# Itseez/opencv

Hardware: AMD Instinct MI355X
Metric: Mpix/s per GPU (4K CV_8U Gaussian5x5) + achieved HBM GB/s vs roofline, 1/2/4/8 GPUs (higher is better)
Workload: dtype u8; 1 GPU; cv::GaussianBlur 5x5 sigma=0 BORDER_REFLECT_101 on 3840x2160 CV_8UC1, 9216 device-resident frames per GPU per step (152.9 GB of HBM: one pass = 18 launches of 512 frames); frames_per_gpu=9216, frames_per_launch=512, ranks=1, collective=none (1 GPU)

## Files before the change

opencv_amd/csrc/smooth.hip:

```cpp
#include "rt.h"
#include "gausskernel.h"
#include "seproll.h"
#include "seplong.h"
#include "sepmx.h"
#include <cstring>
#include <cstdlib>

using namespace mi355;

namespace {

struct FixedTaps { uint16_t kx[33]; uint16_t ky[33]; int nx, ny; };

__global__ __launch_bounds__(256) void k_sepfixed_generic(
    const uchar* __restrict__ src, size_t sstep, size_t sframe,
    uchar* __restrict__ dst, size_t dstep, size_t dframe,
    int W, int H, int cn, int mL, int mT, int mR, int mB, int border, FixedTaps t)
{
    const int b = blockIdx.x * 64 + (threadIdx.x & 63);
    const int y = blockIdx.y * 4 + (threadIdx.x >> 6);
    if (b >= W * cn || y >= H) return;
    src += (size_t)blockIdx.z * sframe;
    dst += (size_t)blockIdx.z * dframe;
    const int x = b / cn, c = b - x * cn;
    const int fullW = mL + W + mR, fullH = mT + H + mB;
    const int rx = t.nx / 2, ry = t.ny / 2;
    uint32_t acc = 0;
    for (int j = 0; j < t.ny; j++) {
        int yy = mi355_borderInterpolate(y + mT + j - ry, fullH, border);
        if (yy < 0) continue;
        const uchar* row = src + (ptrdiff_t)(yy - mT) * (ptrdiff_t)sstep;
        uint32_t h = 0;
        for (int i = 0; i < t.nx; i++) {
            int xx = mi355_borderInterpolate(x + mL + i - rx, fullW, border);
            if (xx < 0) continue;
            h += (uint32_t)t.kx[i] * row[(ptrdiff_t)(xx - mL) * cn + c];
        }
        h = h > 0xFFFFu ? 0xFFFFu : h;
        uint64_t a = (uint64_t)acc + (uint64_t)t.ky[j] * h;
        acc = a > 0xFFFFFFFFull ? 0xFFFFFFFFu : (uint32_t)a;
    }
    uint32_t r = (uint32_t)(((uint64_t)acc + 0x8000u) >> 16);
    dst[(size_t)y * dstep + b] = (uchar)(r > 255 ? 255 : r);
}

constexpr int floordiv2(int a) { return a >= 0 ? a / 2 : -((-a + 1) / 2); }
constexpr int mod2(int a) { return ((a % 2) + 2) % 2; }

template <int Q, int S, int HD>
__device__ __forceinline__ uint32_t pairAt(const uint32_t* E, const uint32_t* O, int k)
{
    constexpr int q2 = mod2(Q + S);
    constexpr int f = floordiv2(Q + S);
    const uint32_t* P = q2 ? O : E;
    if constexpr (mod2(f) == 0) {
        return P[k + f / 2 + HD];
    } else {
        constexpr int lo = floordiv2(f - 1) + 0;
        return __builtin_amdgcn_alignbit(P[k + lo + 1 + HD], P[k + lo + HD], 16);
    }
}

template <int HD> struct RawRow {
    uint4 m;
    uint32_t hl[HD];
    uint32_t hr[HD];
};

template <int KS, int CN> struct RollCfg {
    static constexpr int R = KS / 2;
    static constexpr int HB = R * CN;
    static constexpr int HD = (HB + 3) / 4;
};

template <int KS, int CN>
__device__ __forceinline__ void loadRow(RawRow<RollCfg<KS, CN>::HD>& r, const uchar* __restrict__ src, size_t sstep,
                                        int yy, int W, int H, int c, int nchunks, int lane, int border)
{
    constexpr int HD = RollCfg<KS, CN>::HD, HB = RollCfg<KS, CN>::HB;
    r.m = make_uint4(0, 0, 0, 0);
#pragma unroll
    for (int d = 0; d < HD; d++) { r.hl[d] = 0; r.hr[d] = 0; }
    const int ry = mi355_borderInterpolate(yy, H, border);
    if (ry < 0 || c >= nchunks) return;
    const uchar* row = src + (size_t)ry * sstep;
    r.m = *reinterpret_cast<const uint4*>(row + 16 * (size_t)c);
    if (lane == 0) {
        if (c > 0) {
#pragma unroll
            for (int d = 0; d < HD; d++) r.hl[d] = *reinterpret_cast<const uint32_t*>(row + 16 * (size_t)c - 4 * (HD - d));
        } else {
#pragma unroll
            for (int t = -HB; t < 0; t++) {
                const int px = (t - (CN - 1)) / CN;
                const int ch = t - px * CN;
                const int sp = mi355_borderInterpolate(px, W, border);
                const uint32_t v = sp < 0 ? 0u : row[sp * CN + ch];
                r.hl[(4 * HD + t) >> 2] |= v << (8 * ((4 * HD + t) & 3));
            }
        }
    }
    if (c == nchunks - 1) {
#pragma unroll
        for (int t = 0; t < HB; t++) {
            const int px = W + t / CN, ch = t % CN;
            const int sp = mi355_borderInterpolate(px, W, border);
            const uint32_t v = sp < 0 ? 0u : row[sp * CN + ch];
            r.hr[t >> 2] |= v << (8 * (t & 3));
        }
    } else if (lane == 63) {
#pragma unroll
        for (int d = 0; d < HD; d++) r.hr[d] = *reinterpret_cast<const uint32_t*>(row + 16 * (size_t)c + 16 + 4 * d);
    }
}

template <int KS, int CN>
__device__ __forceinline__ void hfilter(uint32_t (&Hrow)[8], const RawRow<RollCfg<KS, CN>::HD>& r, int c, int nchunks, int lane)
{
    constexpr int HD = RollCfg<KS, CN>::HD;
    constexpr int NW = 4 + 2 * HD;
    uint32_t X[NW];
    const uint32_t mv[4] = {r.m.x, r.m.y, r.m.z, r.m.w};
#pragma unroll
    for (int d = 0; d < HD; d++) {
        uint32_t l = __shfl_up(mv[4 - HD + d], 1);
        uint32_t rr = __shfl_down(mv[d], 1);
        X[d] = (lane == 0) ? r.hl[d] : l;
        X[HD + 4 + d] = (lane == 63 || c == nchunks - 1) ? r.hr[d] : rr;
    }
#pragma unroll
    for (int d = 0; d < 4; d++) X[HD + d] = mv[d];
    uint32_t E[NW], O[NW];
#pragma unroll
    for (int d = 0; d < NW; d++) {
        E[d] = __builtin_amdgcn_perm(0u, X[d], 0x0c020c00u);
        O[d] = __builtin_amdgcn_perm(0u, X[d], 0x0c030c01u);
    }
#pragma unroll
    for (int k = 0; k < 4; k++) {
        if constexpr (KS == 5) {
            {   uint32_t a = pairAt<0, -2 * CN, HD>(E, O, k) + pairAt<0, 2 * CN, HD>(E, O, k);
                uint32_t b = pairAt<0, -CN, HD>(E, O, k) + pairAt<0, CN, HD>(E, O, k);
                uint32_t m = pairAt<0, 0, HD>(E, O, k);
                Hrow[k] = a + (b << 2) + (m << 1) + (m << 2); }
            {   uint32_t a = pairAt<1, -2 * CN, HD>(E, O, k) + pairAt<1, 2 * CN, HD>(E, O, k);
                uint32_t b = pairAt<1, -CN, HD>(E, O, k) + pairAt<1, CN, HD>(E, O, k);
                uint32_t m = pairAt<1, 0, HD>(E, O, k);
                Hrow[4 + k] = a + (b << 2) + (m << 1) + (m << 2); }
        } else {
            Hrow[k]     = pairAt<0, -CN, HD>(E, O, k) + pairAt<0, CN, HD>(E, O, k) + (pairAt<0, 0, HD>(E, O, k) << 1);
            Hrow[4 + k] = pairAt<1, -CN, HD>(E, O, k) + pairAt<1, CN, HD>(E, O, k) + (pairAt<1, 0, HD>(E, O, k) << 1);
        }
    }
}

template <int KS, int CN>
__global__ __launch_bounds__(256) void k_binomial_roll(
    const uchar* __restrict__ src, size_t sstep, size_t sframe,
    uchar* __restrict__ dst, size_t dstep, size_t dframe,
    int W, int H, int nchunks, int segRows, int border)
{
    constexpr int R = KS / 2, HD = RollCfg<KS, CN>::HD;
    const int lane = threadIdx.x & 63;
    const int c = (blockIdx.x * 4 + (threadIdx.x >> 6)) * 64 + lane;
    const int y0 = blockIdx.y * segRows;
    const int y1 = min(H, y0 + segRows);
    src += (size_t)blockIdx.z * sframe;
    dst += (size_t)blockIdx.z * dframe;
    const bool active = c < nchunks;

    uint32_t Hw[KS][8];
    {
        RawRow<HD> pre[KS - 1];
#pragma unroll
        for (int i = 0; i < KS - 1; i++) loadRow<KS, CN>(pre[i], src, sstep, y0 - R + i, W, H, c, nchunks, lane, border);
#pragma unroll
        for (int i = 0; i < KS - 1; i++) hfilter<KS, CN>(Hw[i], pre[i], c, nchunks, lane);
    }
    for (int y = y0; y < y1; y += KS) {
        RawRow<HD> raw[KS];
#pragma unroll
        for (int u = 0; u < KS; u++)
            if (y + u < y1) loadRow<KS, CN>(raw[u], src, sstep, y + u + R, W, H, c, nchunks, lane, border);
#pragma unroll
        for (int u = 0; u < KS; u++) {
            if (y + u < y1) {
                hfilter<KS, CN>(Hw[(KS - 1 + u) % KS], raw[u], c, nchunks, lane);
                uint32_t o[4];
                if constexpr (KS == 5) {
                    const uint32_t* h0 = Hw[(u + 0) % 5]; const uint32_t* h1 = Hw[(u + 1) % 5];
                    const uint32_t* h2 = Hw[(u + 2) % 5]; const uint32_t* h3 = Hw[(u + 3) % 5];
                    const uint32_t* h4 = Hw[(u + 4) % 5];
                    uint32_t v[8];
#pragma unroll
                    for (int i = 0; i < 8; i++) {
                        const uint32_t b4 = lshlAdd(h1[i] + h3[i] + h2[i], 2, 0x00800080u);
                        v[i] = h0[i] + h4[i] + lshlAdd(h2[i], 1, b4);
                    }
#pragma unroll
                    for (int k = 0; k < 4; k++) o[k] = __builtin_amdgcn_perm(v[4 + k], v[k], 0x07030501u);
                } else {
                    const uint32_t* h0 = Hw[(u + 0) % 3]; const uint32_t* h1 = Hw[(u + 1) % 3]; const uint32_t* h2 = Hw[(u + 2) % 3];
#pragma unroll
                    for (int k = 0; k < 4; k++) {
                        uint32_t ve = ((h0[k] + h2[k] + (h1[k] << 1) + 0x00080008u) >> 4) & 0x00FF00FFu;
                        uint32_t vo = ((h0[4 + k] + h2[4 + k] + (h1[4 + k] << 1) + 0x00080008u) >> 4) & 0x00FF00FFu;
                        o[k] = ve | (vo << 8);
                    }
                }
                if (active)
                    *reinterpret_cast<uint4*>(dst + (size_t)(y + u) * dstep + 16 * (size_t)c) = make_uint4(o[0], o[1], o[2], o[3]);
            }
        }
    }
}

template <int HD> struct RawRow2 {
    uint4 m;
    uint32_t side[HD];
};

template <int HD> struct EdgeSel {
    uint32_t la[HD], lb[HD], lc[HD];
    uint32_t ra[HD], rb[HD], rc[HD];
};

__device__ __forceinline__ void selSetByte(uint32_t& a, uint32_t& b, uint32_t& c, int j, int idx )
{
    const uint32_t sh = 8u * (uint32_t)j, clr = ~(0xffu << sh);
    uint32_t va = 0x0cu, vb = 0x0cu, vc = 0x0cu;
    if (idx >= 8)      { vb = (uint32_t)(idx - 8); vc = 4u + (uint32_t)j; }
    else if (idx >= 0) { va = (uint32_t)idx;       vc = (uint32_t)j; }
    a = (a & clr) | (va << sh); b = (b & clr) | (vb << sh); c = (c & clr) | (vc << sh);
}

__device__ __forceinline__ uint32_t gather16(const uint4& m, uint32_t a, uint32_t b, uint32_t c)
{
    const uint32_t t1 = __builtin_amdgcn_perm(m.y, m.x, a);
    const uint32_t t2 = __builtin_amdgcn_perm(m.w, m.z, b);
    return __builtin_amdgcn_perm(t2, t1, c);
}

template <int KS, int CN, bool NTL = false>
__device__ __forceinline__ void issueRow(RawRow2<RollCfg<KS, CN>::HD>& r, const uchar* __restrict__ row, int mainOff, int sideOff)
{
    constexpr int HD = RollCfg<KS, CN>::HD;
    if constexpr (NTL) {
        typedef uint32_t u32x4 __attribute__((ext_vector_type(4)));
        u32x4 v = __builtin_nontemporal_load(reinterpret_cast<const u32x4*>(row + mainOff));
        r.m = make_uint4(v.x, v.y, v.z, v.w);
    } else
    r.m = *reinterpret_cast<const uint4*>(row + mainOff);
#pragma unroll
    for (int d = 0; d < HD; d++) r.side[d] = *reinterpret_cast<const uint32_t*>(row + sideOff + 4 * d);
}

template <int KS, int CN, bool EB = true>
__device__ __forceinline__ void hfilter2(uint32_t (&Hrow)[8], const RawRow2<RollCfg<KS, CN>::HD>& r,
                                         bool hasFirst, bool hasLast, bool isLastChunk, const EdgeSel<RollCfg<KS, CN>::HD>& es)
{
    constexpr int HD = RollCfg<KS, CN>::HD;
    constexpr int NW = 4 + 2 * HD;
    uint32_t X[NW];
    const uint32_t mv[4] = {r.m.x, r.m.y, r.m.z, r.m.w};
    uint32_t hl[HD], hr[HD];
#pragma unroll
    for (int d = 0; d < HD; d++) { hl[d] = r.side[d]; hr[d] = r.side[d]; }
    if (hasFirst) {
#pragma unroll
        for (int d = 0; d < HD; d++) { hl[d] = gather16(r.m, es.la[d], es.lb[d], es.lc[d]); if constexpr (EB) asm volatile("" : "+v"(hl[d])); }
    }
    uint32_t hb[HD];
#pragma unroll
    for (int d = 0; d < HD; d++) hb[d] = 0;
    if (hasLast) {
#pragma unroll
        for (int d = 0; d < HD; d++) { hb[d] = gather16(r.m, es.ra[d], es.rb[d], es.rc[d]); if constexpr (EB) asm volatile("" : "+v"(hb[d])); }
    }
#pragma unroll
    for (int d = 0; d < HD; d++) {
        X[d] = __builtin_amdgcn_update_dpp(hl[d], mv[4 - HD + d], 0x138, 0xf, 0xf, false);
        uint32_t rr = __builtin_amdgcn_update_dpp(hr[d], mv[d], 0x130, 0xf, 0xf, false);
        if (hasLast) { rr = isLastChunk ? hb[d] : rr; if constexpr (EB) asm volatile("" : "+v"(rr)); }
        X[HD + 4 + d] = rr;
    }
#pragma unroll
    for (int d = 0; d < 4; d++) X[HD + d] = mv[d];
    uint32_t E[NW], O[NW];
#pragma unroll
    for (int d = 0; d < NW; d++) {
        E[d] = __builtin_amdgcn_perm(0u, X[d], 0x0c020c00u);
        O[d] = __builtin_amdgcn_perm(0u, X[d], 0x0c030c01u);
    }
#pragma unroll
    for (int k = 0; k < 4; k++) {
        if constexpr (KS == 5) {
            {   uint32_t a = pairAt<0, -2 * CN, HD>(E, O, k) + pairAt<0, 2 * CN, HD>(E, O, k);
                uint32_t b = pairAt<0, -CN, HD>(E, O, k) + pairAt<0, CN, HD>(E, O, k);
                uint32_t m = pairAt<0, 0, HD>(E, O, k);
                Hrow[k] = a + (b << 2) + (m << 1) + (m << 2); }
            {   uint32_t a = pairAt<1, -2 * CN, HD>(E, O, k) + pairAt<1, 2 * CN, HD>(E, O, k);
                uint32_t b = pairAt<1, -CN, HD>(E, O, k) + pairAt<1, CN, HD>(E, O, k);
                uint32_t m = pairAt<1, 0, HD>(E, O, k);
                Hrow[4 + k] = a + (b << 2) + (m << 1) + (m << 2); }
        } else {
            Hrow[k]     = pairAt<0, -CN, HD>(E, O, k) + pairAt<0, CN, HD>(E, O, k) + (pairAt<0, 0, HD>(E, O, k) << 1);
            Hrow[4 + k] = pairAt<1, -CN, HD>(E, O, k) + pairAt<1, CN, HD>(E, O, k) + (pairAt<1, 0, HD>(E, O, k) << 1);
        }
    }
}

template <int KS, int CN, bool NT, bool NTL, int WPS, bool EB = true>
__global__ __launch_bounds__(256, WPS) void k_binomial_roll2(
    const uchar* __restrict__ src, size_t sstep, size_t sframe,
    uchar* __restrict__ dst, size_t dstep, size_t dframe,
    int W, int H, int nchunks, int nstrips, int segRows, int nseg, int nframes, int border, int alt)
{
    constexpr int R = KS / 2, HD = RollCfg<KS, CN>::HD, HB = RollCfg<KS, CN>::HB;
    const int lane = threadIdx.x & 63;
    const int wid = __builtin_amdgcn_readfirstlane((int)(blockIdx.x * 4 + (threadIdx.x >> 6)));
    const int strip = wid % nstrips;
    const int t0 = wid / nstrips;
    int seg = t0 % nseg;
    const int frame = t0 / nseg;
    if (frame >= nframes) return;
    int up = 0;
    if (alt) {
        const int G = 1 << alt, span = 8 * G;
        const int g = seg / span, j = seg - g * span;
        if ((g + 1) * span <= nseg) seg = g * span + G * (j & 7) + (j >> 3);
        else if (alt > 1) {
            const int base = g * span, t = seg - base, g2 = t >> 4, j2 = t & 15;
            if (base + (g2 << 4) + 16 <= nseg) seg = base + (g2 << 4) + 2 * (j2 & 7) + (j2 >> 3);
        }
        up = seg & 1;
    }
    const int c = strip * 64 + lane;
    const int y0 = seg * segRows;
    const int y1 = min(H, y0 + segRows);
    src += (size_t)frame * sframe;
    dst += (size_t)frame * dframe;
    const bool active = c < nchunks;
    const bool hasFirst = strip == 0, hasLast = strip == nstrips - 1;
    const bool isLastChunk = c == nchunks - 1;
    const int ce = active ? c : nchunks - 1;
    const int mainOff = 16 * ce;
    const int c0 = strip * 64;
    const int leftOff = c0 > 0 ? 16 * c0 - 4 * HD : 0;
    const int rightOff = c0 + 64 < nchunks ? 16 * (c0 + 64) : 16 * (nchunks - 1);
    const int sideOff = lane < 32 ? leftOff : rightOff;

    EdgeSel<HD> es;
#pragma unroll
    for (int d = 0; d < HD; d++) { es.la[d] = es.lb[d] = es.lc[d] = es.ra[d] = es.rb[d] = es.rc[d] = 0x0c0c0c0cu; }
    if (hasFirst) {
#pragma unroll
        for (int t = 0; t < HB; t++) {
            const int bt = t - HB;
            const int px = (bt - (CN - 1)) / CN;
            const int sp = mi355_borderInterpolate(px, W, border);
            const int pos = 4 * HD - HB + t;
            selSetByte(es.la[pos >> 2], es.lb[pos >> 2], es.lc[pos >> 2], pos & 3, sp < 0 ? -1 : sp * CN + (bt - px * CN));
        }
    }
    if (hasLast) {
#pragma unroll
        for (int t = 0; t < HB; t++) {
            const int sp = mi355_borderInterpolate(W + t / CN, W, border);
            selSetByte(es.ra[t >> 2], es.rb[t >> 2], es.rc[t >> 2], t & 3, sp < 0 ? -1 : sp * CN + (t % CN) - 16 * (nchunks - 1));
        }
    }
    int rowBelow[R], rowAbove[R];
#pragma unroll
    for (int i = 0; i < R; i++) { rowBelow[i] = mi355_borderInterpolate(H + i, H, border); rowAbove[i] = mi355_borderInterpolate(-1 - i, H, border); }
    const int nrows = y1 - y0;
    auto gy = [&](int j) -> int { return up ? y1 - 1 - j : y0 + j; };
    auto rowIdx = [&](int g) -> int {
        int ry = g;
#pragma unroll
        for (int i = 0; i < R; i++) { ry = (g == H + i) ? rowBelow[i] : ry; ry = (g == -1 - i) ? rowAbove[i] : ry; }
        return ry;
    };

    uint32_t Hw[KS][8];
#pragma unroll
    for (int i = 0; i < KS - 1; i++) {
        const int ry = rowIdx(gy(min(i - R, nrows - 1 + R)));
        if (ry < 0) {
#pragma unroll
            for (int j = 0; j < 8; j++) Hw[i][j] = 0;
        } else {
            RawRow2<HD> pre;
            issueRow<KS, CN>(pre, src + (size_t)ry * sstep, mainOff, sideOff);
            hfilter2<KS, CN, EB>(Hw[i], pre, hasFirst, hasLast, isLastChunk, es);
        }
    }
    RawRow2<HD> raw[KS];
    int rvalid[KS];
#pragma unroll
    for (int u = 0; u < KS; u++) {
        const int ry = rowIdx(gy(min(u + R, nrows - 1 + R)));
        rvalid[u] = ry >= 0;
        issueRow<KS, CN, NTL>(raw[u], src + (size_t)max(ry, 0) * sstep, mainOff, sideOff);
    }
    for (int y = 0; y < nrows; y += KS) {
#pragma unroll
        for (int u = 0; u < KS; u++) {
            if (y + u < nrows) {
                uint32_t (&Hn)[8] = Hw[(KS - 1 + u) % KS];
                if (rvalid[u]) hfilter2<KS, CN, EB>(Hn, raw[u], hasFirst, hasLast, isLastChunk, es);
                else {
#pragma unroll
                    for (int j = 0; j < 8; j++) Hn[j] = 0;
                }
                {
                    const int ry = rowIdx(gy(min(y + u + KS + R, nrows - 1 + R)));
                    rvalid[u] = ry >= 0;
                    issueRow<KS, CN, NTL>(raw[u], src + (size_t)max(ry, 0) * sstep, mainOff, sideOff);
                }
                uint32_t o[4];
                if constexpr (KS == 5) {
                    const uint32_t* h0 = Hw[(u + 0) % 5]; const uint32_t* h1 = Hw[(u + 1) % 5];
                    const uint32_t* h2 = Hw[(u + 2) % 5]; const uint32_t* h3 = Hw[(u + 3) % 5];
                    const uint32_t* h4 = Hw[(u + 4) % 5];
                    uint32_t v[8];
#pragma unroll
                    for (int i = 0; i < 8; i++) {
                        if constexpr (EB) {
                            const uint32_t b4 = lshlAdd(h1[i] + h3[i] + h2[i], 2, 0x00800080u);
                            v[i] = h0[i] + h4[i] + lshlAdd(h2[i], 1, b4);
                        } else
                            v[i] = (h0[i] + h4[i]) + ((h1[i] + h3[i]) << 2) + (h2[i] << 1) + (h2[i] << 2) + 0x00800080u;
                    }
#pragma unroll
                    for (int k = 0; k < 4; k++) o[k] = __builtin_amdgcn_perm(v[4 + k], v[k], 0x07030501u);
                } else {
                    const uint32_t* h0 = Hw[(u + 0) % 3]; const uint32_t* h1 = Hw[(u + 1) % 3]; const uint32_t* h2 = Hw[(u + 2) % 3];
#pragma unroll
                    for (int k = 0; k < 4; k++) {
                        uint32_t ve = ((h0[k] + h2[k] + (h1[k] << 1) + 0x00080008u) >> 4) & 0x00FF00FFu;
                        uint32_t vo = ((h0[4 + k] + h2[4 + k] + (h1[4 + k] << 1) + 0x00080008u) >> 4) & 0x00FF00FFu;
                        o[k] = ve | (vo << 8);
                    }
                }
                if (active) {
                    typedef uint32_t u32x4 __attribute__((ext_vector_type(4)));
                    u32x4 ov = {o[0], o[1], o[2], o[3]};
                    u32x4* dp = reinterpret_cast<u32x4*>(dst + (size_t)gy(y + u) * dstep + 16 * (size_t)c);
                    if constexpr (NT) __builtin_nontemporal_store(ov, dp);
                    else *dp = ov;
                }
            }
        }
    }
}

template <bool NT>
__global__ __launch_bounds__(256) void k_copy16(const uint4* __restrict__ s, uint4* __restrict__ d, size_t n16, int perThread)
{
    typedef uint32_t u32x4 __attribute__((ext_vector_type(4)));
    size_t base = ((size_t)blockIdx.x * perThread) * 256 + threadIdx.x;
#pragma unroll 4
    for (int i = 0; i < perThread; i++) {
        size_t j = base + (size_t)i * 256;
        if (j < n16) {
            uint4 v = s[j];
            u32x4 ov = {v.x, v.y, v.z, v.w};
            if constexpr (NT) __builtin_nontemporal_store(ov, reinterpret_cast<u32x4*>(d + j));
            else d[j] = v;
        }
    }
}

template <int UNROLL>
__global__ __launch_bounds__(256) void k_copy_colwalk(const uchar* __restrict__ src, uchar* __restrict__ dst, size_t step, size_t frame,
                                                      int H, int nchunks, int nstrips, int segRows, int nseg, int nframes)
{
    const int lane = threadIdx.x & 63;
    const int wid = __builtin_amdgcn_readfirstlane((int)(blockIdx.x * 4 + (threadIdx.x >> 6)));
    const int strip = wid % nstrips, t0 = wid / nstrips, seg = t0 % nseg, fr = t0 / nseg;
    if (fr >= nframes) return;
    const int c = strip * 64 + lane;
    if (c >= nchunks) return;
    const int y0 = seg * segRows, y1 = min(H, y0 + segRows);
    const uchar* s = src + (size_t)fr * frame + 16 * (size_t)c;
    uchar* d = dst + (size_t)fr * frame + 16 * (size_t)c;
    for (int y = y0; y < y1; y += UNROLL) {
        uint4 v[UNROLL];
#pragma unroll
        for (int u = 0; u < UNROLL; u++) v[u] = *reinterpret_cast<const uint4*>(s + (size_t)min(y + u, y1 - 1) * step);
#pragma unroll
        for (int u = 0; u < UNROLL; u++) if (y + u < y1) *reinterpret_cast<uint4*>(d + (size_t)(y + u) * step) = v[u];
    }
}


bool aligned16(const void* p, size_t step) { return (((uintptr_t)p | step) & 15) == 0; }

int envInt(const char* n, int d) { const char* v = getenv(n); return v ? atoi(v) : d; }

int& tuneSeg() { static int v = envInt("MI355CV_GAUSS_SEG", 0); return v; }
int& tuneVariant() { static int v = envInt("MI355CV_GAUSS_VARIANT", 3); return v; }

int& tuneAlt() { static int v = envInt("MI355CV_GAUSS_ALT", 1); return v; }
int& tuneLaunchWaves() { static int v = envInt("MI355CV_GAUSS_LAUNCH_WAVES", 393216); return v; }

template <int KS, int CN>
void launchRoll2(const uchar* s, size_t ss, size_t sf, uchar* d, size_t ds, size_t df, int nframes, int W, int H, int border, hipStream_t st, int nt)
{
    const int nchunks = W * CN / 16;
    const int nstrips = divUp(nchunks, 64);
    int seg = tuneSeg();
    if (seg <= 0) {
        long long per = (long long)nstrips * nframes;
        long long wantSeg = (2048 + per - 1) / per;
        seg = (int)((H + wantSeg - 1) / wantSeg);
        const int best = 16;
        if (seg > best) seg = best;
        if (seg < KS) seg = KS;
    }
    if (seg > H) seg = H;
    const int nseg = divUp(H, seg);
    const long long perFrame = (long long)nstrips * nseg;
    long long chunk = tuneLaunchWaves() > 0 ? (tuneLaunchWaves() + perFrame - 1) / perFrame : nframes;
    if (chunk < 1) chunk = 1;
    if (chunk > nframes) chunk = nframes;
    const int nlaunch = (int)((nframes + chunk - 1) / chunk);
    noteKernel("k_binomial_roll2<%d,%d,%s,false,%d,%s> grid=%u x256 seg=%d rows alt=%d, %d launch(es) of <= %lld frames", KS, CN, nt >= 1 ? "true" : "false", nt == 3 ? 6 : 4,
               nt == 2 ? "false" : "true", (unsigned)((perFrame * chunk + 3) / 4), seg, tuneAlt(), nlaunch, chunk);
    for (long long f0 = 0; f0 < nframes; f0 += chunk) {
        const int nf = (int)(nframes - f0 < chunk ? nframes - f0 : chunk);
        const uchar* sp = s + (size_t)f0 * sf;
        uchar* dp = d + (size_t)f0 * df;
        dim3 grid((unsigned)((perFrame * nf + 3) / 4));
        if (nt == 3)      hipLaunchKernelGGL((k_binomial_roll2<KS, CN, true, false, 6>), grid, dim3(256), 0, st, sp, ss, sf, dp, ds, df, W, H, nchunks, nstrips, seg, nseg, nf, border, tuneAlt());
        else if (nt == 2) hipLaunchKernelGGL((k_binomial_roll2<KS, CN, true, false, 4, false>), grid, dim3(256), 0, st, sp, ss, sf, dp, ds, df, W, H, nchunks, nstrips, seg, nseg, nf, border, tuneAlt());
        else if (nt == 1) hipLaunchKernelGGL((k_binomial_roll2<KS, CN, true, false, 4>), grid, dim3(256), 0, st, sp, ss, sf, dp, ds, df, W, H, nchunks, nstrips, seg, nseg, nf, border, tuneAlt());
        else              hipLaunchKernelGGL((k_binomial_roll2<KS, CN, false, false, 4>), grid, dim3(256), 0, st, sp, ss, sf, dp, ds, df, W, H, nchunks, nstrips, seg, nseg, nf, border, tuneAlt());
    }
}

template <int KS, int CN>
void launchRoll(const uchar* s, size_t ss, size_t sf, uchar* d, size_t ds, size_t df, int nframes, int W, int H, int border, hipStream_t st)
{
    const int nchunks = W * CN / 16;
    const int gx = divUp(nchunks, 256);
    const int segEnv = tuneSeg();
    int seg;
    if (segEnv > 0) seg = segEnv;
    else {
        long long stripsWaves = (long long)divUp(nchunks, 64) * nframes;
        long long wantSeg = (16384 + stripsWaves - 1) / stripsWaves;
        if (wantSeg < 1) wantSeg = 1;
        seg = (int)((H + wantSeg - 1) / wantSeg);
        if (seg < 4 * KS) seg = 4 * KS;
    }
    seg = divUp(seg, KS) * KS;
    if (seg > H) seg = divUp(H, KS) * KS;
    dim3 grid(gx, divUp(H, seg), nframes);
    hipLaunchKernelGGL((k_binomial_roll<KS, CN>), grid, dim3(256), 0, st, s, ss, sf, d, ds, df, W, H, nchunks, seg, border);
}

bool rollEligible(const uchar* s, size_t ss, size_t sf, const uchar* d, size_t ds, size_t df, int W, int H, int cn, int ks)
{
    if (ks != 3 && ks != 5) return false;
    if (cn < 1 || cn > 4) return false;
    if (!aligned16(s, ss) || !aligned16(d, ds) || (sf & 15) || (df & 15)) return false;
    if ((W * cn) % 16 != 0) return false;
    if (H < 1) return false;
    return true;
}

static int sepmxMinTaps()
{
    static const int v = std::getenv("MI355CV_SEPMX_MIN_TAPS") ? atoi(std::getenv("MI355CV_SEPMX_MIN_TAPS")) : 7;
    return v;
}

int runSmooth(const char* entry, const uchar* src, size_t sstep, size_t sframe, uchar* dst, size_t dstep, size_t dframe,
              int nframes, int W, int H, int cn, int mL, int mT, int mR, int mB,
              const uint16_t* kx, int nx, const uint16_t* ky, int ny, int border, bool binomial)
{
    if (disabled()) return mi355::declined(__func__, __LINE__, "disabled()");
    if (W <= 0 || H <= 0 || nframes <= 0 || cn < 1 || cn > 4) return mi355::declined(__func__, __LINE__, "W <= 0 || H <= 0 || nframes <= 0 || cn < 1 || cn > 4");
    if (nx < 1 || ny < 1 || nx > lim::GAUSS8U_MAX_KSIZE || ny > lim::GAUSS8U_MAX_KSIZE || !(nx & 1) || !(ny & 1)) return mi355::declined(__func__, __LINE__, "nx < 1 || ny < 1 || nx or ny > lim::GAUSS8U_MAX_KSIZE || !(nx & 1) || !(ny & 1)");
    if (border < 0 || border > B_REFLECT_101) return mi355::declined(__func__, __LINE__, "border < 0 || border > B_REFLECT_101");
    Stager stg;
    if (!ensureDevice()) return mi355::declined(__func__, __LINE__, "!ensureDevice()");
    const bool hostSrc = !isDevicePtr(src);
    if (hostSrc && (size_t)W * H < minPixels()) return mi355::declined(__func__, __LINE__, "hostSrc && (size_t)W * H < minPixels()");
    if (!hostSrc && src == dst) return mi355::declined(__func__, __LINE__, "!hostSrc && src == dst");

    size_t dss = 0, dds = 0;
    const size_t rowB = (size_t)W * cn;
    const uchar* dsrc; uchar* ddst;
    if (nframes == 1) {
        const uchar* top = src - (ptrdiff_t)mT * (ptrdiff_t)sstep - (ptrdiff_t)mL * cn;
        const uchar* dtop = stg.in(top, sstep, (size_t)(mL + W + mR) * cn, mT + H + mB, &dss);
        if (!dtop) return mi355::declined(__func__, __LINE__, "!dtop");
        dsrc = dtop + (size_t)mT * dss + (size_t)mL * cn;
        ddst = stg.out(dst, dstep, rowB, H, &dds);
        if (!ddst) return mi355::declined(__func__, __LINE__, "!ddst");
    } else {
        if (hostSrc || !isDevicePtr(dst)) return setError(MI355CV_NOT_IMPLEMENTED, "%s: batch entry needs device-resident frames", entry);
        dsrc = src; ddst = dst; dss = sstep; dds = dstep;
    }
    hipStream_t st = stream();
    const bool noMargins = !(mL | mT | mR | mB);
    if (binomial && noMargins && rollEligible(dsrc, dss, sframe, ddst, dds, dframe, W, H, cn, nx) && nx == ny) {
#define ROLL(KS_, CN_) do { if (tuneVariant() <= 1 || border == B_WRAP || W <= KS_ / 2) launchRoll<KS_, CN_>(dsrc, dss, sframe, ddst, dds, dframe, nframes, W, H, border, st); \
                            else launchRoll2<KS_, CN_>(dsrc, dss, sframe, ddst, dds, dframe, nframes, W, H, border, st, tuneVariant() - 2); } while (0)
        if (nx == 5) { switch (cn) { case 1: ROLL(5, 1); break; case 2: ROLL(5, 2); break; case 3: ROLL(5, 3); break; default: ROLL(5, 4); } }
        else         { switch (cn) { case 1: ROLL(3, 1); break; case 2: ROLL(3, 2); break; case 3: ROLL(3, 3); break; default: ROLL(3, 4); } }
#undef ROLL
    } else if (std::getenv("MI355CV_SMOOTH_GENERIC") == nullptr && std::max(nx, ny) >= sepmxMinTaps() && !(std::getenv("MI355CV_SEPMX") && std::getenv("MI355CV_SEPMX")[0] == '0') &&
               sepmxRun(stg, dsrc, dss, sframe, ddst, dds, dframe, nframes, W, H, cn, mL + W + mR, mT + H + mB, mL, mT, border, kx, nx, nx / 2, ky, ny, ny / 2, st)) {
    } else if (noMargins && std::getenv("MI355CV_SMOOTH_GENERIC") == nullptr &&
               seprollFixedSmooth(dsrc, dss, sframe, ddst, dds, dframe, nframes, W, H, cn, kx, nx, ky, ny, border, st)) {
    } else if (!noMargins && nframes == 1 && std::getenv("MI355CV_SMOOTH_GENERIC") == nullptr && [&] {
                   const Roi roi = {mL + W + mR, mT + H + mB, mL, mT};
                   return seprollFixedSmooth(dsrc, dss, 0, ddst, dds, 0, 1, W, H, cn, kx, nx, ky, ny, border, st, &roi); }()) {
    } else if (std::getenv("MI355CV_SMOOTH_GENERIC") == nullptr && std::max(nx, ny) < sepmxMinTaps() && !(std::getenv("MI355CV_SEPMX") && std::getenv("MI355CV_SEPMX")[0] == '0') &&
               sepmxRun(stg, dsrc, dss, sframe, ddst, dds, dframe, nframes, W, H, cn, mL + W + mR, mT + H + mB, mL, mT, border, kx, nx, nx / 2, ky, ny, ny / 2, st)) {
    } else if (std::getenv("MI355CV_SMOOTH_GENERIC") == nullptr && [&] {
                   unsigned sx = 0, sy = 0;
                   for (int i = 0; i < nx; i++) sx += kx[i];
                   for (int i = 0; i < ny; i++) sy += ky[i];
                   if (sx > 256 || sy > 256) return false;
                   std::vector<int> ix(kx, kx + nx), iy(ky, ky + ny);
                   const SepLongTaps t = {nullptr, nullptr, ix.data(), iy.data(), nx, ny, nx / 2, ny / 2, 3, 0, 0.f, 0};
                   return seplongRun(stg, dsrc, dss, sframe, ddst, dds, dframe, nframes, W, H, cn, MI355CV_8U, MI355CV_8U, mL + W + mR, mT + H + mB, mL, mT, border, t, st); }()) {
    } else {
        if (nx > 33 || ny > 33) return mi355::declined(__func__, __LINE__, "Q8.8 taps that sum beyond 256 with more than 33 of them");
        FixedTaps t;
        t.nx = nx; t.ny = ny;
        for (int i = 0; i < 33; i++) { t.kx[i] = i < nx ? kx[i] : 0; t.ky[i] = i < ny ? ky[i] : 0; }
        dim3 grid(divUp(W * cn, 64), divUp(H, 4), nframes);
        hipLaunchKernelGGL(k_sepfixed_generic, grid, dim3(256), 0, st, dsrc, dss, sframe, ddst, dds, dframe,
                           W, H, cn, mL, mT, mR, mB, border, t);
    }
    return stg.finish(entry);
}

template <int K>
__global__ __launch_bounds__(256) void k_binom16_direct(const uchar* __restrict__ parent, size_t sstep, uchar* __restrict__ dst, size_t dstep, int W, int H, int cn,
                                                        int mL, int mT, int fullW, int fullH, int border)
{
    constexpr int R = K / 2, SH = K == 3 ? 2 : K == 5 ? 4 : K == 7 ? 6 : 8;
    constexpr uint32_t TAP[9] = {K == 3 ? 1u : K == 5 ? 1u : K == 7 ? 2u : 4u, K == 3 ? 2u : K == 5 ? 4u : K == 7 ? 7u : 13u, K == 3 ? 1u : K == 5 ? 6u : K == 7 ? 14u : 30u,
                                 K == 5 ? 4u : K == 7 ? 18u : 51u, K == 5 ? 1u : K == 7 ? 14u : 60u, K == 7 ? 7u : 51u, K == 7 ? 2u : 30u, 13u, 4u};
    const int e = blockIdx.x * 64 + (threadIdx.x & 63), y = blockIdx.y * 4 + (threadIdx.x >> 6);
    if (e >= W * cn || y >= H) return;
    const int x = e / cn, c = e - x * cn;
    int xs[K];
#pragma unroll
    for (int i = 0; i < K; i++) { const int q = mi355_borderInterpolate(x + mL + i - R, fullW, border); xs[i] = q < 0 ? -1 : q * cn + c; }
    uint32_t acc = 0;
#pragma unroll
    for (int j = 0; j < K; j++) {
        const int q = mi355_borderInterpolate(y + mT + j - R, fullH, border);
        if (q < 0) continue;
        const unsigned short* row = reinterpret_cast<const unsigned short*>(parent + (size_t)q * sstep);
        uint32_t h = 0;
#pragma unroll
        for (int i = 0; i < K; i++) h += xs[i] < 0 ? 0u : TAP[i] * (uint32_t)row[xs[i]];
        acc += TAP[j] * h;
    }
    reinterpret_cast<unsigned short*>(dst + (size_t)y * dstep)[e] = (unsigned short)((acc + (1u << (2 * SH - 1))) >> (2 * SH));
}

int runBinom16(const char* entry, const uchar* src, size_t sstep, uchar* dst, size_t dstep, int W, int H, int cn, int mL, int mT, int mR, int mB, int ksize, int border)
{
    if (disabled() || W <= 0 || H <= 0 || cn < 1 || cn > 4 || (ksize != 3 && ksize != 5 && ksize != 7 && ksize != 9) || border < 0 || border > B_REFLECT_101 ||
        mL < 0 || mT < 0 || mR < 0 || mB < 0 || ((sstep | dstep | (uintptr_t)src | (uintptr_t)dst) & 1))
        return mi355::declined(__func__, __LINE__, "disabled() || W <= 0 || H <= 0 || cn < 1 || cn > 4 || ksize not in {3, 5, 7, 9} || border outside CONSTANT .. REFLECT_101 || negative margins || odd pointers / steps");
    Stager stg;
    if (!ensureDevice()) return mi355::declined(__func__, __LINE__, "!ensureDevice()");
    const bool hostSrc = !isDevicePtr(src);
    if (hostSrc && (size_t)W * H < minPixels()) return mi355::declined(__func__, __LINE__, "hostSrc && (size_t)W * H < minPixels()");
    if (!hostSrc && src == dst) return mi355::declined(__func__, __LINE__, "!hostSrc && src == dst");
    size_t dss = 0, dds = 0;
    const size_t esz = (size_t)cn * 2;
    const uchar* top = src - (ptrdiff_t)mT * (ptrdiff_t)sstep - (ptrdiff_t)mL * (ptrdiff_t)esz;
    const uchar* dtop = stg.in(top, sstep, (size_t)(mL + W + mR) * esz, mT + H + mB, &dss);
    if (!dtop) return mi355::declined(__func__, __LINE__, "!dtop");
    const uchar* dsrc = dtop + (size_t)mT * dss + (size_t)mL * esz;
    uchar* ddst = stg.out(dst, dstep, (size_t)W * esz, H, &dds);
    if (!ddst) return mi355::declined(__func__, __LINE__, "!ddst");
    const Roi roi = {mL + W + mR, mT + H + mB, mL, mT};
    if (cn == 1 && (ksize == 3 || ksize == 5) && border != B_WRAP &&
        seprollBinom16(dsrc, dss, 0, ddst, dds, 0, 1, W, H, ksize, border, stream(), (mL | mT | mR | mB) ? &roi : nullptr))
// ... 214 lines not shown
```

Measured before the change: 2.947 million Mpix/s.

## Add specialized fast path for rolling binomial kernel without border validity checks

Adds a fast path to the rolling separable binomial kernel for the common case: interior segments, or any non-constant border. In that path rows never need zero-fill, so the per-row validity tracking is dropped. The loop is split into steady-state, tail and remainder phases with scheduling barriers, and interior strips use an edge-free hfilter instantiation. Inactive lanes now exit early, and offsets are pinned as 32-bit VGPR values via empty asm so addressing stays cheap. The cost is more code size and register pressure, and the sched barriers may limit how well the compiler overlaps loads with ALU work.

```diff
diff --git a/opencv_amd/csrc/smooth.hip b/opencv_amd/csrc/smooth.hip
--- a/opencv_amd/csrc/smooth.hip
+++ b/opencv_amd/csrc/smooth.hip
@@ -5,6 +5,7 @@
 #include "sepmx.h"
 #include <cstring>
 #include <cstdlib>
+#include <type_traits>
 
 using namespace mi355;
 
@@ -242,9 +243,10 @@
 }
 
 template <int KS, int CN, bool NTL = false>
-__device__ __forceinline__ void issueRow(RawRow2<RollCfg<KS, CN>::HD>& r, const uchar* __restrict__ row, int mainOff, int sideOff)
+__device__ __forceinline__ void issueRow(RawRow2<RollCfg<KS, CN>::HD>& r, const uchar* __restrict__ row, uint32_t mainOff, uint32_t sideOff)
 {
     constexpr int HD = RollCfg<KS, CN>::HD;
+    asm volatile("" : "+v"(mainOff), "+v"(sideOff));
     if constexpr (NTL) {
         typedef uint32_t u32x4 __attribute__((ext_vector_type(4)));
         u32x4 v = __builtin_nontemporal_load(reinterpret_cast<const u32x4*>(row + mainOff));
@@ -308,6 +310,46 @@
             Hrow[4 + k] = pairAt<1, -CN, HD>(E, O, k) + pairAt<1, CN, HD>(E, O, k) + (pairAt<1, 0, HD>(E, O, k) << 1);
         }
     }
+}
+
+template <int KS, bool EB>
+__device__ __forceinline__ void vfilter2(uint32_t (&o)[4], const uint32_t (&Hw)[KS][8], int u)
+{
+    if constexpr (KS == 5) {
+        const uint32_t* h0 = Hw[(u + 0) % 5]; const uint32_t* h1 = Hw[(u + 1) % 5];
+        const uint32_t* h2 = Hw[(u + 2) % 5]; const uint32_t* h3 = Hw[(u + 3) % 5];
+        const uint32_t* h4 = Hw[(u + 4) % 5];
+        uint32_t v[8];
+#pragma unroll
+        for (int i = 0; i < 8; i++) {
+            if constexpr (EB) {
+                const uint32_t b4 = lshlAdd(h1[i] + h3[i] + h2[i], 2, 0x00800080u);
+                v[i] = h0[i] + h4[i] + lshlAdd(h2[i], 1, b4);
+            } else
+                v[i] = (h0[i] + h4[i]) + ((h1[i] + h3[i]) << 2) + (h2[i] << 1) + (h2[i] << 2) + 0x00800080u;
+        }
+#pragma unroll
+        for (int k = 0; k < 4; k++) o[k] = __builtin_amdgcn_perm(v[4 + k], v[k], 0x07030501u);
+    } else {
+        const uint32_t* h0 = Hw[(u + 0) % 3]; const uint32_t* h1 = Hw[(u + 1) % 3]; const uint32_t* h2 = Hw[(u + 2) % 3];
+#pragma unroll
+        for (int k = 0; k < 4; k++) {
+            uint32_t ve = ((h0[k] + h2[k] + (h1[k] << 1) + 0x00080008u) >> 4) & 0x00FF00FFu;
+            uint32_t vo = ((h0[4 + k] + h2[4 + k] + (h1[4 + k] << 1) + 0x00080008u) >> 4) & 0x00FF00FFu;
+            o[k] = ve | (vo << 8);
+        }
+    }
+}
+
+template <bool NT>
+__device__ __forceinline__ void storeRow(uchar* row, uint32_t off, const uint32_t (&o)[4])
+{
+    typedef uint32_t u32x4 __attribute__((ext_vector_type(4)));
+    u32x4 ov = {o[0], o[1], o[2], o[3]};
+    asm volatile("" : "+v"(off));
+    uchar* p = row + off;
+    if constexpr (NT) __builtin_nontemporal_store(ov, reinterpret_cast<u32x4*>(p));
+    else *reinterpret_cast<u32x4*>(p) = ov;
 }
 
 template <int KS, int CN, bool NT, bool NTL, int WPS, bool EB = true>
@@ -340,15 +382,14 @@
     const int y1 = min(H, y0 + segRows);
     src += (size_t)frame * sframe;
     dst += (size_t)frame * dframe;
-    const bool active = c < nchunks;
+    if (c >= nchunks) return;
     const bool hasFirst = strip == 0, hasLast = strip == nstrips - 1;
     const bool isLastChunk = c == nchunks - 1;
-    const int ce = active ? c : nchunks - 1;
-    const int mainOff = 16 * ce;
+    const uint32_t mainOff = 16u * (uint32_t)c;
     const int c0 = strip * 64;
     const int leftOff = c0 > 0 ? 16 * c0 - 4 * HD : 0;
     const int rightOff = c0 + 64 < nchunks ? 16 * (c0 + 64) : 16 * (nchunks - 1);
-    const int sideOff = lane < 32 ? leftOff : rightOff;
+    const uint32_t sideOff = (uint32_t)(lane < 32 ? leftOff : rightOff);
 
     EdgeSel<HD> es;
 #pragma unroll
@@ -383,6 +424,51 @@
     };
 
     uint32_t Hw[KS][8];
+    RawRow2<HD> raw[KS];
+
+    auto rowPtr = [&](int j) -> const uchar* { return src + (size_t)rowIdx(gy(j)) * sstep; };
+    auto fastPath = [&](auto edgeTag) {
+        constexpr bool EDGE = decltype(edgeTag)::value;
+        const bool eF = EDGE && hasFirst, eL = EDGE && hasLast, eC = EDGE && isLastChunk;
+        auto rowStep = [&](int u, int j, bool refill) {
+            hfilter2<KS, CN, false>(Hw[(KS - 1 + u) % KS], raw[u], eF, eL, eC, es);
+            if (refill) issueRow<KS, CN, NTL>(raw[u], rowPtr(j + KS + R), mainOff, sideOff);
+            uint32_t o[4];
+            vfilter2<KS, EB>(o, Hw, u);
+            storeRow<NT>(dst + (size_t)gy(j) * dstep, mainOff, o);
+            __builtin_amdgcn_sched_barrier(0);
+        };
+        {
+            RawRow2<HD> pre[KS - 1];
+#pragma unroll
+            for (int i = 0; i < KS - 1; i++) issueRow<KS, CN>(pre[i], rowPtr(i - R), mainOff, sideOff);
+#pragma unroll
+            for (int u = 0; u < KS; u++)
+                if (u < nrows) issueRow<KS, CN, NTL>(raw[u], rowPtr(u + R), mainOff, sideOff);
+#pragma unroll
+            for (int i = 0; i < KS - 1; i++) hfilter2<KS, CN, false>(Hw[i], pre[i], eF, eL, eC, es);
+        }
+        int y = 0;
+        for (; y + 2 * KS <= nrows; y += KS) {
+#pragma unroll
+            for (int u = 0; u < KS; u++) rowStep(u, y + u, true);
+        }
+        if (y + KS <= nrows) {
+            const int left = nrows - y - KS;
+#pragma unroll
+            for (int u = 0; u < KS; u++) rowStep(u, y + u, u < left);
+            y += KS;
+        }
+#pragma unroll
+        for (int u = 0; u < KS - 1; u++)
+            if (y + u < nrows) rowStep(u, y + u, false);
+    };
+    if ((y0 >= R && y1 + R <= H) || border != B_CONSTANT) {
+        if (hasFirst || hasLast) fastPath(std::true_type());
+        else fastPath(std::false_type());
+        return;
+    }
+
 #pragma unroll
     for (int i = 0; i < KS - 1; i++) {
         const int ry = rowIdx(gy(min(i - R, nrows - 1 + R)));
@@ -395,7 +481,6 @@
             hfilter2<KS, CN, EB>(Hw[i], pre, hasFirst, hasLast, isLastChunk, es);
         }
     }
-    RawRow2<HD> raw[KS];
     int rvalid[KS];
 #pragma unroll
     for (int u = 0; u < KS; u++) {
@@ -419,37 +504,8 @@
                     issueRow<KS, CN, NTL>(raw[u], src + (size_t)max(ry, 0) * sstep, mainOff, sideOff);
                 }
                 uint32_t o[4];
-                if constexpr (KS == 5) {
-                    const uint32_t* h0 = Hw[(u + 0) % 5]; const uint32_t* h1 = Hw[(u + 1) % 5];
-                    const uint32_t* h2 = Hw[(u + 2) % 5]; const uint32_t* h3 = Hw[(u + 3) % 5];
-                    const uint32_t* h4 = Hw[(u + 4) % 5];
-                    uint32_t v[8];
-#pragma unroll
-                    for (int i = 0; i < 8; i++) {
-                        if constexpr (EB) {
-                            const uint32_t b4 = lshlAdd(h1[i] + h3[i] + h2[i], 2, 0x00800080u);
-                            v[i] = h0[i] + h4[i] + lshlAdd(h2[i], 1, b4);
-                        } else
-                            v[i] = (h0[i] + h4[i]) + ((h1[i] + h3[i]) << 2) + (h2[i] << 1) + (h2[i] << 2) + 0x00800080u;
-                    }
-#pragma unroll
-                    for (int k = 0; k < 4; k++) o[k] = __builtin_amdgcn_perm(v[4 + k], v[k], 0x07030501u);
-                } else {
-                    const uint32_t* h0 = Hw[(u + 0) % 3]; const uint32_t* h1 = Hw[(u + 1) % 3]; const uint32_t* h2 = Hw[(u + 2) % 3];
-#pragma unroll
-                    for (int k = 0; k < 4; k++) {
-                        uint32_t ve = ((h0[k] + h2[k] + (h1[k] << 1) + 0x00080008u) >> 4) & 0x00FF00FFu;
-                        uint32_t vo = ((h0[4 + k] + h2[4 + k] + (h1[4 + k] << 1) + 0x00080008u) >> 4) & 0x00FF00FFu;
-                        o[k] = ve | (vo << 8);
-                    }
-                }
-                if (active) {
-                    typedef uint32_t u32x4 __attribute__((ext_vector_type(4)));
-                    u32x4 ov = {o[0], o[1], o[2], o[3]};
-                    u32x4* dp = reinterpret_cast<u32x4*>(dst + (size_t)gy(y + u) * dstep + 16 * (size_t)c);
-                    if constexpr (NT) __builtin_nontemporal_store(ov, dp);
-                    else *dp = ov;
-                }
+                vfilter2<KS, EB>(o, Hw, u);
+                storeRow<NT>(dst + (size_t)gy(y + u) * dstep, mainOff, o);
             }
         }
     }
```

Result: no change. 2.925 million Mpix/s (-0.7%).

## Add steady-state row loop specialized by strip edge position for binomial roll kernel

Applied to the files above, without the earlier changes.

Adds an opt-in steady mode (nt==4) that specializes the rolling 5x5 binomial kernel by strip edge type: interior, first or last strip. Each specialization runs an inner-row loop without per-row border index lookups and validity checks, using pointer increments and a buffer store with bounds clipping for the last strip. The vertical filter is factored into a helper function. The aim is to cut per-row scalar and branch overhead, at the cost of more code (four kernel instantiations) and possible register pressure.

```diff
diff --git a/opencv_amd/csrc/smooth.hip b/opencv_amd/csrc/smooth.hip
--- a/opencv_amd/csrc/smooth.hip
+++ b/opencv_amd/csrc/smooth.hip
@@ -310,11 +310,42 @@
     }
 }
 
+template <int KS, bool EB>
+__device__ __forceinline__ void vfilter2(uint32_t (&o)[4], const uint32_t (&Hw)[KS][8], int u)
+{
+    if constexpr (KS == 5) {
+        const uint32_t* h0 = Hw[(u + 0) % 5]; const uint32_t* h1 = Hw[(u + 1) % 5];
+        const uint32_t* h2 = Hw[(u + 2) % 5]; const uint32_t* h3 = Hw[(u + 3) % 5];
+        const uint32_t* h4 = Hw[(u + 4) % 5];
+        uint32_t v[8];
+#pragma unroll
+        for (int i = 0; i < 8; i++) {
+            if constexpr (EB) {
+                const uint32_t b4 = lshlAdd(h1[i] + h3[i] + h2[i], 2, 0x00800080u);
+                v[i] = h0[i] + h4[i] + lshlAdd(h2[i], 1, b4);
+            } else
+                v[i] = (h0[i] + h4[i]) + ((h1[i] + h3[i]) << 2) + (h2[i] << 1) + (h2[i] << 2) + 0x00800080u;
+        }
+#pragma unroll
+        for (int k = 0; k < 4; k++) o[k] = __builtin_amdgcn_perm(v[4 + k], v[k], 0x07030501u);
+    } else {
+        const uint32_t* h0 = Hw[(u + 0) % 3]; const uint32_t* h1 = Hw[(u + 1) % 3]; const uint32_t* h2 = Hw[(u + 2) % 3];
+#pragma unroll
+        for (int k = 0; k < 4; k++) {
+            uint32_t ve = ((h0[k] + h2[k] + (h1[k] << 1) + 0x00080008u) >> 4) & 0x00FF00FFu;
+            uint32_t vo = ((h0[4 + k] + h2[4 + k] + (h1[4 + k] << 1) + 0x00080008u) >> 4) & 0x00FF00FFu;
+            o[k] = ve | (vo << 8);
+        }
+    }
+}
+
+template <int V> struct IntTag { static constexpr int value = V; };
+
 template <int KS, int CN, bool NT, bool NTL, int WPS, bool EB = true>
 __global__ __launch_bounds__(256, WPS) void k_binomial_roll2(
     const uchar* __restrict__ src, size_t sstep, size_t sframe,
     uchar* __restrict__ dst, size_t dstep, size_t dframe,
-    int W, int H, int nchunks, int nstrips, int segRows, int nseg, int nframes, int border, int alt)
+    int W, int H, int nchunks, int nstrips, int segRows, int nseg, int nframes, int border, int alt, int steady)
 {
     constexpr int R = KS / 2, HD = RollCfg<KS, CN>::HD, HB = RollCfg<KS, CN>::HB;
     const int lane = threadIdx.x & 63;
@@ -350,10 +381,14 @@
     const int rightOff = c0 + 64 < nchunks ? 16 * (c0 + 64) : 16 * (nchunks - 1);
     const int sideOff = lane < 32 ? leftOff : rightOff;
 
+    auto item = [&](auto edge) __attribute__((always_inline)) {
+    constexpr int EDGE = decltype(edge)::value;
+    const bool hF = EDGE == 0 ? hasFirst : EDGE == 2, hL = EDGE == 0 ? hasLast : EDGE == 3;
+    const bool act = (EDGE == 1 || EDGE == 2) ? true : active;
     EdgeSel<HD> es;
 #pragma unroll
     for (int d = 0; d < HD; d++) { es.la[d] = es.lb[d] = es.lc[d] = es.ra[d] = es.rb[d] = es.rc[d] = 0x0c0c0c0cu; }
-    if (hasFirst) {
+    if (hF) {
 #pragma unroll
         for (int t = 0; t < HB; t++) {
             const int bt = t - HB;
@@ -363,7 +398,7 @@
             selSetByte(es.la[pos >> 2], es.lb[pos >> 2], es.lc[pos >> 2], pos & 3, sp < 0 ? -1 : sp * CN + (bt - px * CN));
         }
     }
-    if (hasLast) {
+    if (hL) {
 #pragma unroll
         for (int t = 0; t < HB; t++) {
             const int sp = mi355_borderInterpolate(W + t / CN, W, border);
@@ -392,7 +427,7 @@
         } else {
             RawRow2<HD> pre;
             issueRow<KS, CN>(pre, src + (size_t)ry * sstep, mainOff, sideOff);
-            hfilter2<KS, CN, EB>(Hw[i], pre, hasFirst, hasLast, isLastChunk, es);
+            hfilter2<KS, CN, EB>(Hw[i], pre, hF, hL, isLastChunk, es);
         }
     }
     RawRow2<HD> raw[KS];
@@ -403,12 +438,52 @@
         rvalid[u] = ry >= 0;
         issueRow<KS, CN, NTL>(raw[u], src + (size_t)max(ry, 0) * sstep, mainOff, sideOff);
     }
-    for (int y = 0; y < nrows; y += KS) {
+    int y = 0;
+    if constexpr (EDGE != 0) {
+        const int jLast = nrows - 1 + R, jImg = up ? y1 - 1 : H - 1 - y0;
+        int ssEnd = nrows / KS * KS;
+        if (jLast > jImg) { const int t = jImg - (2 * KS - 1 + R); ssEnd = t < 0 ? 0 : min(ssEnd, (t / KS + 1) * KS); }
+        if (nrows < 2 * KS) ssEnd = 0;
+        if (ssEnd > 0) {
+            const ptrdiff_t sinc = up ? -(ptrdiff_t)sstep : (ptrdiff_t)sstep, dinc = up ? -(ptrdiff_t)dstep : (ptrdiff_t)dstep;
+            const uchar* pf = src + (size_t)gy(KS + R) * sstep;
+            uchar* dq = dst + (size_t)gy(0) * dstep;
+            int jn = KS + R;
+            auto trip = [&]() __attribute__((always_inline)) {
+#pragma unroll
+                for (int u = 0; u < KS; u++) {
+                    hfilter2<KS, CN, EB>(Hw[(KS - 1 + u) % KS], raw[u], hF, hL, isLastChunk, es);
+                    issueRow<KS, CN, NTL>(raw[u], pf, mainOff, sideOff);
+                    {   const bool adv = jn < jLast;
+                        pf += adv ? sinc : 0; jn += adv ? 1 : 0; }
+                    uint32_t o[4];
+                    vfilter2<KS, EB>(o, Hw, u);
+                    typedef uint32_t u32x4 __attribute__((ext_vector_type(4)));
+                    u32x4 ov = {o[0], o[1], o[2], o[3]};
+                    if constexpr (EDGE == 3) {
+                        __builtin_amdgcn_raw_buffer_store_b128(ov, __builtin_amdgcn_make_buffer_rsrc(dq, 0, 16 * nchunks, 0x00020000), 16 * c, 0, NT ? 2 : 0);
+                    } else {
+                        u32x4* dp = reinterpret_cast<u32x4*>(dq + 16 * (size_t)c);
+                        if constexpr (NT) __builtin_nontemporal_store(ov, dp);
+                        else *dp = ov;
+                    }
+                    dq += dinc;
+                    __builtin_amdgcn_sched_barrier(0);
+                }
+                y += KS;
+            };
+            trip();
+            while (y < ssEnd) trip();
+#pragma unroll
+            for (int u = 0; u < KS; u++) rvalid[u] = 1;
+        }
+    }
+    for (; y < nrows; y += KS) {
 #pragma unroll
         for (int u = 0; u < KS; u++) {
             if (y + u < nrows) {
                 uint32_t (&Hn)[8] = Hw[(KS - 1 + u) % KS];
-                if (rvalid[u]) hfilter2<KS, CN, EB>(Hn, raw[u], hasFirst, hasLast, isLastChunk, es);
+                if (rvalid[u]) hfilter2<KS, CN, EB>(Hn, raw[u], hF, hL, isLastChunk, es);
                 else {
 #pragma unroll
                     for (int j = 0; j < 8; j++) Hn[j] = 0;
@@ -419,31 +494,8 @@
                     issueRow<KS, CN, NTL>(raw[u], src + (size_t)max(ry, 0) * sstep, mainOff, sideOff);
                 }
                 uint32_t o[4];
-                if constexpr (KS == 5) {
-                    const uint32_t* h0 = Hw[(u + 0) % 5]; const uint32_t* h1 = Hw[(u + 1) % 5];
-                    const uint32_t* h2 = Hw[(u + 2) % 5]; const uint32_t* h3 = Hw[(u + 3) % 5];
-                    const uint32_t* h4 = Hw[(u + 4) % 5];
-                    uint32_t v[8];
-#pragma unroll
-                    for (int i = 0; i < 8; i++) {
-                        if constexpr (EB) {
-                            const uint32_t b4 = lshlAdd(h1[i] + h3[i] + h2[i], 2, 0x00800080u);
-                            v[i] = h0[i] + h4[i] + lshlAdd(h2[i], 1, b4);
-                        } else
-                            v[i] = (h0[i] + h4[i]) + ((h1[i] + h3[i]) << 2) + (h2[i] << 1) + (h2[i] << 2) + 0x00800080u;
-                    }
-#pragma unroll
-                    for (int k = 0; k < 4; k++) o[k] = __builtin_amdgcn_perm(v[4 + k], v[k], 0x07030501u);
-                } else {
-                    const uint32_t* h0 = Hw[(u + 0) % 3]; const uint32_t* h1 = Hw[(u + 1) % 3]; const uint32_t* h2 = Hw[(u + 2) % 3];
-#pragma unroll
-                    for (int k = 0; k < 4; k++) {
-                        uint32_t ve = ((h0[k] + h2[k] + (h1[k] << 1) + 0x00080008u) >> 4) & 0x00FF00FFu;
-                        uint32_t vo = ((h0[4 + k] + h2[4 + k] + (h1[4 + k] << 1) + 0x00080008u) >> 4) & 0x00FF00FFu;
-                        o[k] = ve | (vo << 8);
-                    }
-                }
-                if (active) {
+                vfilter2<KS, EB>(o, Hw, u);
+                if (act) {
                     typedef uint32_t u32x4 __attribute__((ext_vector_type(4)));
                     u32x4 ov = {o[0], o[1], o[2], o[3]};
                     u32x4* dp = reinterpret_cast<u32x4*>(dst + (size_t)gy(y + u) * dstep + 16 * (size_t)c);
@@ -453,6 +505,14 @@
             }
         }
     }
+    };
+    if constexpr (NT && EB && WPS == 4) {
+        if (!steady || (hasFirst && hasLast)) item(IntTag<0>{});
+        else if (hasFirst) item(IntTag<2>{});
+        else if (hasLast)  item(IntTag<3>{});
+        else               item(IntTag<1>{});
+    } else
+        item(IntTag<0>{});
 }
 
 template <bool NT>
@@ -526,6 +586,8 @@
     if (chunk < 1) chunk = 1;
     if (chunk > nframes) chunk = nframes;
     const int nlaunch = (int)((nframes + chunk - 1) / chunk);
+    const int steady = nt == 4;
+    if (steady) nt = 1;
     noteKernel("k_binomial_roll2<%d,%d,%s,false,%d,%s> grid=%u x256 seg=%d rows alt=%d, %d launch(es) of <= %lld frames", KS, CN, nt >= 1 ? "true" : "false", nt == 3 ? 6 : 4,
                nt == 2 ? "false" : "true", (unsigned)((perFrame * chunk + 3) / 4), seg, tuneAlt(), nlaunch, chunk);
     for (long long f0 = 0; f0 < nframes; f0 += chunk) {
@@ -533,10 +595,10 @@
         const uchar* sp = s + (size_t)f0 * sf;
         uchar* dp = d + (size_t)f0 * df;
         dim3 grid((unsigned)((perFrame * nf + 3) / 4));
-        if (nt == 3)      hipLaunchKernelGGL((k_binomial_roll2<KS, CN, true, false, 6>), grid, dim3(256), 0, st, sp, ss, sf, dp, ds, df, W, H, nchunks, nstrips, seg, nseg, nf, border, tuneAlt());
-        else if (nt == 2) hipLaunchKernelGGL((k_binomial_roll2<KS, CN, true, false, 4, false>), grid, dim3(256), 0, st, sp, ss, sf, dp, ds, df, W, H, nchunks, nstrips, seg, nseg, nf, border, tuneAlt());
-        else if (nt == 1) hipLaunchKernelGGL((k_binomial_roll2<KS, CN, true, false, 4>), grid, dim3(256), 0, st, sp, ss, sf, dp, ds, df, W, H, nchunks, nstrips, seg, nseg, nf, border, tuneAlt());
-        else              hipLaunchKernelGGL((k_binomial_roll2<KS, CN, false, false, 4>), grid, dim3(256), 0, st, sp, ss, sf, dp, ds, df, W, H, nchunks, nstrips, seg, nseg, nf, border, tuneAlt());
+        if (nt == 3)      hipLaunchKernelGGL((k_binomial_roll2<KS, CN, true, false, 6>), grid, dim3(256), 0, st, sp, ss, sf, dp, ds, df, W, H, nchunks, nstrips, seg, nseg, nf, border, tuneAlt(), 0);
+        else if (nt == 2) hipLaunchKernelGGL((k_binomial_roll2<KS, CN, true, false, 4, false>), grid, dim3(256), 0, st, sp, ss, sf, dp, ds, df, W, H, nchunks, nstrips, seg, nseg, nf, border, tuneAlt(), 0);
+        else if (nt == 1) hipLaunchKernelGGL((k_binomial_roll2<KS, CN, true, false, 4>), grid, dim3(256), 0, st, sp, ss, sf, dp, ds, df, W, H, nchunks, nstrips, seg, nseg, nf, border, tuneAlt(), steady);
+        else              hipLaunchKernelGGL((k_binomial_roll2<KS, CN, false, false, 4>), grid, dim3(256), 0, st, sp, ss, sf, dp, ds, df, W, H, nchunks, nstrips, seg, nseg, nf, border, tuneAlt(), 0);
     }
 }
 
```

Measured after the change: 2.957 million Mpix/s before, 2.802 million Mpix/s after. 0.948x the previous value.
